# microsoft/DirectXTex

Hardware: AMD Instinct MI355X
Metric: Mtexels/s BC7 encode (4096^2 RGBA8, TEX_COMPRESS_DEFAULT) (higher is better)
Workload: dtype fp32 seed fit + i32 exact error sums (u8 texels in, 128-bit blocks out); 1 GPU; cfg2: 4096x4096 RGBA8 -> BC7_UNORM, TEX_COMPRESS_DEFAULT, one image per GPU, source and payload resident in HBM (dxtex_compress_device)

## Files before the change

directxtex_amd/csrc/bc6h_encode.hip:

```cpp
#include "dxtex_kernels.h"
#include "bc67_tables.h"
#include "bc7_core.h"
#include "bc6h_core.h"
#include "search_common.h"
#include <algorithm>
#include <cstdlib>
#include <cstdio>
#include <vector>

namespace dxtex
{
namespace
{
using namespace bc6h;

struct Ep16 { uint32_t a01, a2b0, b12; };
__device__ __forceinline__ Ep16 pack_ep16(const int (&A)[3], const int (&B)[3])
{
    Ep16 e;
    e.a01 = (uint32_t(A[0]) & 0xFFFFu) | (uint32_t(A[1]) << 16);
    e.a2b0 = (uint32_t(A[2]) & 0xFFFFu) | (uint32_t(B[0]) << 16);
    e.b12 = (uint32_t(B[1]) & 0xFFFFu) | (uint32_t(B[2]) << 16);
    return e;
}
// ... 24 lines not shown
    return s;
}
struct Rec6 { Ep16 ep; float err; };
struct Best6 { float err; uint32_t mode; uint64_t lo, hi; };
struct OrgSave { Ep16 ep; float err; uint64_t idx; };
struct OptSave { uint64_t idx; float err; uint32_t swapped; };

enum : int { SEED_INTS = 17 * 6 + 2 };

struct Bc6hArgs
{
    SegTable seg;
    uint32_t nblocks;
    int isSigned;
    int prune;
    uint32_t taskBase;
    int prec1[4];
    float* fpix;
    uint8_t* lists;
    int* seeds;
    Rec6* recs;
    OrgSave* orgs;
    uint2* order; uint32_t* tinfo; uint32_t* counters;
    Best6* best;
    float* bounds;
    int boundsReady;
    int filterStats;
    int samePrec;
    struct OptSave* opts;
    int saveOpt;
    ModeRt mode;
};

constexpr uint32_t kDoneBit6 = 1u << 23;

#if !defined(DXTEX_BC6H_DEFAULT_ORDER)
#define DXTEX_BC6H_DEFAULT_ORDER "5,6,7,8,0,2,3,4,1,9"
#endif

__device__ __forceinline__ Texels slot_texels(float* slot , int np)
{
    Texels t; t.r = slot; t.g = slot + 16 * 64; t.b = slot + 32 * 64; t.stride = 64; t.np = np;
    return t;
}

__device__ __forceinline__ int gather_texels(const float* planes, uint32_t mask, float* slot, uint64_t& pos)
// ... 921 lines not shown
        if (lane == 0)
        {
            a.recs[myTask].ep = pack_ep16(st.ep.A, st.ep.B);
            { const float mk = ep16_mark(sg, st.ep.A, st.ep.B); if (mk < 0.0f) a.recs[myTask].err = mk; }
        }
    }
}

__global__ void __launch_bounds__(256) bc6h_store_kernel(Bc6hArgs a)
{
    const uint32_t nb = blockIdx.x * 256u + threadIdx.x;
    if (nb >= a.nblocks) return;
    const Best6 b = a.best[nb];
    const BcSeg& im = seg_of(a.seg, nb);
    const uint32_t gb = im.nb0 + (nb - im.l0);
    const uint32_t by = gb / im.nbw, bx = gb - by * im.nbw;
    uint64_t* out = reinterpret_cast<uint64_t*>(im.dst + uint64_t(by) * im.dstRowPitch) + 2 * uint64_t(bx);
    out[0] = b.lo; out[1] = b.hi;
}

const uint64_t kMaxBlocksPerPass6 = dev_env("DXTEX_MAX_BLOCKS_PER_PASS") ? std::max<uint64_t>(1, strtoull(dev_env("DXTEX_MAX_BLOCKS_PER_PASS"), nullptr, 10)) : (1u << 22);
struct Scratch6
{
    size_t fpix, lists, seeds, recs, orgs, order, tinfo, counters, best, bounds, recs1, orgs1, order1, tinfo1, counters1, opts, total;
    explicit Scratch6(uint64_t nb)
    {
        auto up = [](size_t v) { return (v + 255) & ~size_t(255); };
        size_t o = 0;
        fpix = o; o = up(o + nb * 48 * sizeof(float));
        lists = o; o = up(o + nb * 8);
        seeds = o; o = up(o + nb * SEED_INTS * sizeof(int));
        recs = o; o = up(o + nb * 16 * sizeof(Rec6));
        orgs = o; o = up(o + nb * 16 * sizeof(OrgSave));
        order = o; o = up(o + nb * 16 * sizeof(uint2));
        tinfo = o; o = up(o + nb * 16 * sizeof(uint32_t));
        counters = o; o = up(o + 128 * sizeof(uint32_t));
        best = o; o = up(o + nb * sizeof(Best6));
        bounds = o; o = up(o + nb * 17 * sizeof(float));
        recs1 = o; o = up(o + nb * 4 * sizeof(Rec6));
        orgs1 = o; o = up(o + nb * 4 * sizeof(OrgSave));
        order1 = o; o = up(o + nb * 4 * sizeof(uint2));
        tinfo1 = o; o = up(o + nb * 4 * sizeof(uint32_t));
        counters1 = o; o = up(o + 128 * sizeof(uint32_t));
        opts = o; o = up(o + nb * 16 * sizeof(OptSave));
        total = o;
    }
};
}

size_t bc6h_scratch_bytes(uint64_t nblocks, size_t nimages)
{
    return Scratch6(nblocks < kMaxBlocksPerPass6 ? nblocks : kMaxBlocksPerPass6).total + seg_table_bytes(nblocks, kMaxBlocksPerPass6, nimages);
}

hipError_t launch_bc6h_encode(const SrcView& src, uint8_t* dst, uint64_t dstRowPitch, bool isSigned, void* scratch,
                              hipStream_t stream, KernelMarks* marks, const SideStreams* side)
{
    BcImage one; one.src = src; one.dst = dst; one.dstRowPitch = dstRowPitch;
    return launch_bc6h_encode_many(&one, 1, isSigned, scratch, stream, marks, side);
}

hipError_t launch_bc6h_encode_many(const BcImage* images, size_t count, bool isSigned, void* scratch, hipStream_t stream, KernelMarks* marks,
                                   const SideStreams* side)
{
#define DXTEX_MARK(NAME) do { if (marks) marks->mark(NAME); } while (0)
    std::vector<BcSeg> segs;
// ... 1 lines not shown
    uint64_t perPass = 0;
    if (!build_passes(images, count, kMaxBlocksPerPass6, segs, passes, &perPass)) return hipSuccess;
    const Scratch6 L(perPass);
    uint8_t* base = static_cast<uint8_t*>(scratch);
    BcSeg* dSegs = reinterpret_cast<BcSeg*>(base + L.total);
    const hipError_t ce = upload_segments(dSegs, segs, passes, stream);
    if (ce != hipSuccess) return ce;
    for (const BcPass& pass : passes)
    {
        Bc6hArgs a;
        set_pass(a.seg, dSegs, segs, pass);
        a.nblocks = pass.nblocks;
        a.isSigned = isSigned ? 1 : 0;
        static const bool noPrune = dev_env("DXTEX_BC6H_NO_PRUNE") != nullptr;
        a.prune = noPrune ? 0 : 1;
        a.fpix = reinterpret_cast<float*>(base + L.fpix);
        a.lists = base + L.lists;
        a.seeds = reinterpret_cast<int*>(base + L.seeds);
        a.recs = reinterpret_cast<Rec6*>(base + L.recs);
        a.orgs = reinterpret_cast<OrgSave*>(base + L.orgs);
        a.order = reinterpret_cast<uint2*>(base + L.order);
        a.tinfo = reinterpret_cast<uint32_t*>(base + L.tinfo);
        a.counters = reinterpret_cast<uint32_t*>(base + L.counters);
        a.best = reinterpret_cast<Best6*>(base + L.best);
        a.bounds = reinterpret_cast<float*>(base + L.bounds);
        a.opts = reinterpret_cast<OptSave*>(base + L.opts);
        a.saveOpt = 0;
        a.boundsReady = 0;
        a.filterStats = 0;
        a.mode = ModeRt();

        DXTEX_MARK("bc6h_rough");
        hipLaunchKernelGGL(bc6h_rough_kernel, dim3((a.nblocks + 3) / 4), dim3(256), 0, stream, a);
        DXTEX_MARK("bc6h_block_seed");
        hipLaunchKernelGGL(bc6h_block_seed_kernel, dim3((a.nblocks + 255) / 256), dim3(256), 0, stream, a);
        if (dev_env("DXTEX_BC6H_DUMP"))
        {
            (void)hipStreamSynchronize(stream);
            const uint32_t n = std::min<uint32_t>(a.nblocks, 4);
            std::vector<uint8_t> l(n * 8); std::vector<int> sd(n * SEED_INTS);
            (void)hipMemcpy(l.data(), a.lists, l.size(), hipMemcpyDeviceToHost);
            (void)hipMemcpy(sd.data(), a.seeds, sd.size() * 4, hipMemcpyDeviceToHost);
            for (uint32_t b = 0; b < n; ++b)
            {
                fprintf(stderr, "block %u shapes:", b);
                for (int i = 0; i < 8; ++i) fprintf(stderr, " %d", l[b * 8 + i]);
                fprintf(stderr, "\n  seeds rank0:");
                for (int i = 0; i < 12; ++i) fprintf(stderr, " %d", sd[b * SEED_INTS + i]);
                fprintf(stderr, "\n");
            }
        }
        static const int onlyMode = dev_env("DXTEX_BC6H_ONLY_MODE") ? atoi(dev_env("DXTEX_BC6H_ONLY_MODE")) : -1;
        static const bool noSearch = dev_env("DXTEX_BC6H_NO_SEARCH") != nullptr;
        static const Bc6hMode kModes[14] = {
            { 0x00, 1, 1, 3, { 10, 10, 10 }, { 5, 5, 5 } }, { 0x01, 1, 1, 3, { 7, 7, 7 }, { 6, 6, 6 } }, { 0x02, 1, 1, 3, { 11, 11, 11 }, { 5, 4, 4 } },
            { 0x06, 1, 1, 3, { 11, 11, 11 }, { 4, 5, 4 } }, { 0x0a, 1, 1, 3, { 11, 11, 11 }, { 4, 4, 5 } }, { 0x0e, 1, 1, 3, { 9, 9, 9 }, { 5, 5, 5 } },
            { 0x12, 1, 1, 3, { 8, 8, 8 }, { 6, 5, 5 } }, { 0x16, 1, 1, 3, { 8, 8, 8 }, { 5, 6, 5 } }, { 0x1a, 1, 1, 3, { 8, 8, 8 }, { 5, 5, 6 } },
            { 0x1e, 1, 0, 3, { 6, 6, 6 }, { 6, 6, 6 } }, { 0x03, 0, 0, 4, { 10, 10, 10 }, { 10, 10, 10 } }, { 0x07, 0, 1, 4, { 11, 11, 11 }, { 9, 9, 9 } },
            { 0x0b, 0, 1, 4, { 12, 12, 12 }, { 8, 8, 8 } }, { 0x0f, 0, 1, 4, { 16, 16, 16 }, { 4, 4, 4 } } };
        auto set_mode_on = [&](Bc6hArgs& a, int mi)
        {
            const Bc6hMode& k = kModes[mi];
            a.mode.index = mi; a.mode.code = k.code; a.mode.regions2 = k.regions2; a.mode.transformed = k.transformed; a.mode.prec = k.prec[0];
            for (int c = 0; c < 3; ++c) a.mode.delta[c] = k.delta[c];
        };
        auto set_mode = [&](int mi) { set_mode_on(a, mi); };
        auto sort_tasks = [&](const Bc6hArgs& a, uint32_t ntasks, hipStream_t stream)
        {
            const uint32_t binGroups = std::min<uint32_t>(kBinGroups, (ntasks + 255) / 256);
            (void)hipMemsetAsync(a.counters, 0, 128 * sizeof(uint32_t), stream);
            hipLaunchKernelGGL(bc7_bin_count_kernel, dim3(binGroups), dim3(256), 0, stream, a.tinfo, ntasks, a.counters);
            hipLaunchKernelGGL(bc7_bin_scan_kernel, dim3(1), dim3(1), 0, stream, a.counters);
            hipLaunchKernelGGL(bc7_bin_scatter_kernel, dim3(binGroups), dim3(256), 0, stream, a.tinfo, ntasks, a.counters, a.order);
        };
        a.taskBase = 0;
        for (int m = 0; m < 4; ++m) a.prec1[m] = kModes[10 + m].prec[0];
        static const std::vector<int> order6 = []
        {
            std::vector<int> o;
            const char* e = dev_env("DXTEX_BC6H_ORDER");
            const char* p = e ? e : DXTEX_BC6H_DEFAULT_ORDER;
            while (*p) { if (*p >= '0' && *p <= '9') o.push_back(int(strtol(p, const_cast<char**>(&p), 10))); else ++p; }
            return o;
        }();
        int prevPrec = -1;
        a.samePrec = 0;
        std::vector<int> run2;
        for (int mi : order6) if (mi >= 0 && mi <= 9 && (onlyMode < 0 || mi == onlyMode)) run2.push_back(mi);
        static const int forkBack = dev_env("DXTEX_BC6H_FORK_BACK") ? atoi(dev_env("DXTEX_BC6H_FORK_BACK")) : 2;
        const SideStreams* fork = (marks || forkBack <= 0 || run2.size() < size_t(forkBack) + 1 || onlyMode >= 0) ? nullptr : side;
        Bc6hArgs a1 = a;
        a1.recs = reinterpret_cast<Rec6*>(base + L.recs1);
        a1.orgs = reinterpret_cast<OrgSave*>(base + L.orgs1);
        a1.order = reinterpret_cast<uint2*>(base + L.order1);
        a1.tinfo = reinterpret_cast<uint32_t*>(base + L.tinfo1);
        a1.counters = reinterpret_cast<uint32_t*>(base + L.counters1);
        a1.samePrec = 0;
        auto one_region_search = [&](hipStream_t stream, KernelMarks* marks)
        {
            const uint32_t gridPP = (a1.nblocks + 255) / 256;
            DXTEX_MARK("bc6h_pre_1region");
            a1.boundsReady = 0;
            for (int m = 0; m < 4; ++m)
            {
                if (onlyMode >= 0 && 10 + m != onlyMode) continue;
                set_mode_on(a1, 10 + m); a1.taskBase = uint32_t(m) * a1.nblocks;
                hipLaunchKernelGGL(bc6h_pre_kernel<0>, dim3(gridPP), dim3(256), 0, stream, a1);
                a1.boundsReady = 1;
            }
            const uint32_t ntasks = a1.nblocks * 4u;
            if (onlyMode >= 0)
                for (int m = 0; m < 4; ++m) if (10 + m != onlyMode) (void)hipMemsetAsync(a1.tinfo + uint64_t(m) * a1.nblocks, 0, uint64_t(a1.nblocks) * 4, stream);
            DXTEX_MARK("bc6h_bin_1region");
            sort_tasks(a1, ntasks, stream);
            DXTEX_MARK("bc6h_perturb_1region");
            static const uint32_t waveMax = dev_env("DXTEX_BC6H_WAVE_MAX") ? uint32_t(strtoul(dev_env("DXTEX_BC6H_WAVE_MAX"), nullptr, 0)) : kWaveTaskMax6;
            if (!noSearch)
            {
                hipLaunchKernelGGL(bc6h_perturb_kernel<16>, dim3(std::min<uint32_t>(kSearchWaves, (ntasks + 63) / 64)), dim3(64), 0, stream, a1, waveMax);
                hipLaunchKernelGGL(bc6h_perturb_wave_kernel, dim3(std::min<uint32_t>(kSearchWaves, ntasks)), dim3(64), 0, stream, a1, waveMax);
            }
        };
        bool forked = false;
        for (size_t at = 0; at < run2.size(); ++at)
        {
            const int mi = run2[at];
            if (fork && at + size_t(forkBack) == run2.size())
            {
                (void)hipEventRecord(fork->forked, stream);
                (void)hipStreamWaitEvent(fork->side[0], fork->forked, 0);
                one_region_search(fork->side[0], nullptr);
                (void)hipEventRecord(fork->joined[0], fork->side[0]);
                forked = true;
            }
            set_mode(mi);
            static const bool noReuse = dev_env("DXTEX_BC6H_NO_REUSE") != nullptr;
            a.samePrec = (!noReuse && prevPrec == kModes[mi].prec[0]) ? 1 : 0;
            prevPrec = kModes[mi].prec[0];
            a.saveOpt = (!noReuse && at + 1 < run2.size() && kModes[run2[at + 1]].prec[0] == kModes[mi].prec[0]) ? 1 : 0;
            const uint32_t ntasks = a.nblocks * 16u;
            const uint32_t gridPP = (a.nblocks + 15) / 16;
            static const char* const kPre[10] = { "bc6h_pre_m0", "bc6h_pre_m1", "bc6h_pre_m2", "bc6h_pre_m3", "bc6h_pre_m4", "bc6h_pre_m5", "bc6h_pre_m6", "bc6h_pre_m7", "bc6h_pre_m8", "bc6h_pre_m9" };
            static const char* const kPerturb[10] = { "bc6h_perturb_m0", "bc6h_perturb_m1", "bc6h_perturb_m2", "bc6h_perturb_m3", "bc6h_perturb_m4", "bc6h_perturb_m5", "bc6h_perturb_m6", "bc6h_perturb_m7", "bc6h_perturb_m8", "bc6h_perturb_m9" };
            static const char* const kPost[10] = { "bc6h_post_m0", "bc6h_post_m1", "bc6h_post_m2", "bc6h_post_m3", "bc6h_post_m4", "bc6h_post_m5", "bc6h_post_m6", "bc6h_post_m7", "bc6h_post_m8", "bc6h_post_m9" };
            DXTEX_MARK(kPre[mi]);
            hipLaunchKernelGGL(bc6h_pre_kernel<1>, dim3(gridPP), dim3(256), 0, stream, a);
            a.boundsReady = 1;
            DXTEX_MARK("bc6h_bin_2region");
            sort_tasks(a, ntasks, stream);
#if defined(DXTEX_DEV)
            static const bool stats6 = dev_env("DXTEX_BC6H_STATS") != nullptr;
            a.filterStats = stats6 ? 1 : 0;
            if (stats6)
            {
                uint32_t c[40] = {};
                (void)hipStreamSynchronize(stream);
                (void)hipMemcpy(c, a.counters, sizeof(c), hipMemcpyDeviceToHost);
                std::fprintf(stderr, "bc6h stats mode %d (prec %d): %u task slots, %u live (16-texel: %u)\n", mi, a.mode.prec, ntasks, c[34], c[16]);
            }
#endif
            DXTEX_MARK(kPerturb[mi]);
            static const bool plainPerturb = dev_env("DXTEX_BC6H_PERTURB_PLAIN") != nullptr;
            if (!noSearch)
            {
                const dim3 grid(std::min<uint32_t>(kSearchWaves, (ntasks + 63) / 64));
                if (plainPerturb) hipLaunchKernelGGL(bc6h_perturb_kernel<8>, grid, dim3(64), 0, stream, a, 0u);
                else if (isSigned) hipLaunchKernelGGL(bc6h_perturb_filter_kernel<true>, grid, dim3(64), 0, stream, a);
                else hipLaunchKernelGGL(bc6h_perturb_filter_kernel<false>, grid, dim3(64), 0, stream, a);
            }
#if defined(DXTEX_DEV)
            if (stats6 && !plainPerturb)
            {
// ... 41 lines not shown
```

directxtex_amd/csrc/bc7_encode.hip:

```cpp
#include "dxtex_kernels.h"
#include "bc67_tables.h"
#include "bc7_core.h"
#include "search_common.h"
#include <algorithm>
#include <cstdio>
#include <cstdlib>
#include <vector>

namespace dxtex
{
namespace
{
using namespace bc7;

struct Cand { uint32_t err; uint32_t ord; uint64_t lo, hi; };

enum : int { SLOT_M0 = 0, SLOT_M1, SLOT_M2, SLOT_M3, SLOT_M4A, SLOT_M4B, SLOT_M5, SLOT_M6, SLOT_M7, NUM_SLOTS };
enum : int { LIST_BYTES = 64 };

enum : int { PHASE_ALL = 0, PHASE_EARLY = 1, PHASE_LATE = 2 };

struct Bc7Args
{
    SegTable seg;
    uint32_t nblocks;
    uint32_t flags;
    uint8_t* lists;
    Cand* cands;
    uint32_t* px;
    struct TaskRec* recs;
    uint2* order;
    uint32_t* tinfo;
    uint32_t* counters;
    uint32_t* zeroOrd;
    uint2* seeds1;
    uint2* seeds3;
    uint2* seeds;
    int* bestErr;
    int prune;
    const uint32_t* flagged;
    uint32_t early6Min;
    uint32_t earlyAlphaMin;
    int early6Pct;
    int phase;
    const uint32_t* gate;
    uint32_t gateMin;
    uint32_t perturbWaveMax;
    uint32_t exhWaveMax;
};

constexpr uint32_t kWaveTaskMax = 262144;
constexpr uint32_t kWaveTaskMax45 = 24576;
constexpr uint32_t kPerturbWaveMax = 32768;

__device__ __forceinline__ void load_block_texel(const SrcView& src, uint32_t nbw, uint32_t nb, uint32_t t, float* f4, uint32_t& ldr)
{
// ... 336 lines not shown
template<int MODE, int IM>
__device__ __forceinline__ void search_pickup(const Bc7Args& a, uint2 task, uint32_t* slotCol, SlotRegion& rg)
{
    typedef TaskMap<MODE, IM> TM;
    const uint32_t nb = task.x / TM::TPB;
    const uint32_t mask = task.y & 0xFFFFu, rot = (task.y >> 16) & 3u;
    const uint4* px4 = reinterpret_cast<const uint4*>(a.px + uint64_t(nb) * 16);
    const uint4 q0 = px4[0], q1 = px4[1], q2 = px4[2], q3 = px4[3];
    const uint32_t px[16] = { q0.x, q0.y, q0.z, q0.w, q1.x, q1.y, q1.z, q1.w, q2.x, q2.y, q2.z, q2.w, q3.x, q3.y, q3.z, q3.w };
    int np = 0;
    if (TM::NS == 1)
    {
#pragma unroll
        for (int i = 0; i < 16; ++i) slotCol[i * kSlotStride] = rotate_pixel(px[i], rot);
        np = 16;
    }
    else
    {
#pragma unroll
        for (int i = 0; i < 16; ++i)
            if ((mask >> i) & 1u) { slotCol[np * kSlotStride] = px[i]; ++np; }
    }
    rg.base = slotCol; rg.np = np; rg.p2sum = 0;
}

__device__ __forceinline__ int lanes_below(unsigned long long mask)
{
    return int(__builtin_amdgcn_mbcnt_hi(uint32_t(mask >> 32), __builtin_amdgcn_mbcnt_lo(uint32_t(mask), 0u)));
}

#if defined(DXTEX_BC7_WAVETIMES)
enum : int { WT_KINDS = 3, WT_KEYS = WT_KINDS * 8 * 2 * 3, WT_FIELDS = 6 };
__device__ unsigned long long g_wt[WT_KEYS][8192][WT_FIELDS];
__device__ unsigned int g_wtHist[WT_KEYS][256];
#define WT_BEGIN(KIND) const int wtKey = (((KIND) * 8 + MODE) * 2 + IM) * 3 + CHSET; const bool wtOn = a.phase != PHASE_EARLY; \
    const unsigned long long wt0 = wall_clock64(); unsigned long long wtDr = 0, wtRounds = 0, wtLanes = 0, wtTasks = 0; int wtMine = 0
#define WT_TAKE(IDX) do { wtTasks += (unsigned long long)__popcll(__ballot((IDX) != 0xFFFFFFFFu)); if (!wtDr && q.drained) wtDr = wall_clock64(); } while (0)
#define WT_ROUND(BUSYL) do { ++wtRounds; wtLanes += (unsigned long long)__popcll(__ballot(BUSYL)); if (BUSYL) ++wtMine; } while (0)
#define WT_DONE() do { wtMine = 0; } while (0)
#define WT_END() do { if (wtOn && lane == 0 && wtRounds) { unsigned long long* w_ = g_wt[wtKey][blockIdx.x & 8191]; w_[0] = wt0; w_[1] = wtDr ? wtDr : wall_clock64(); \
    w_[2] = wall_clock64(); w_[3] = wtRounds; w_[4] = wtLanes; w_[5] = wtTasks; } } while (0)
#else
#define WT_BEGIN(KIND) do { } while (0)
#define WT_TAKE(IDX) do { } while (0)
#define WT_ROUND(BUSYL) do { } while (0)
#define WT_DONE() do { } while (0)
#define WT_END() do { } while (0)
#endif
#if !defined(DXTEX_FLAT_SKIP)
#define DXTEX_FLAT_SKIP 1
#endif
// ... 840 lines not shown
    {
        if (!((slotMask >> s) & 1u)) continue;
        if (s == SLOT_M7 && a.flagged[1] == 0) continue;
        const Cand v = c[s];
        if (v.err == 0xFFFFFFFFu) continue;
        const uint64_t key = (uint64_t(v.err) << 32) | v.ord;
        if (key < bestKey) { bestKey = key; lo = v.lo; hi = v.hi; }
    }
    const BcSeg& sg = seg_of(a.seg, nb);
    const uint32_t gb = sg.nb0 + (nb - sg.l0);
    const uint32_t by = gb / sg.nbw, bx = gb - by * sg.nbw;
    uint64_t* out = reinterpret_cast<uint64_t*>(sg.dst + uint64_t(by) * sg.dstRowPitch) + 2 * uint64_t(bx);
    out[0] = lo; out[1] = hi;
}
}

namespace
{
const uint64_t kMaxBlocksPerPass = dev_env("DXTEX_MAX_BLOCKS_PER_PASS") ? std::max<uint64_t>(1, strtoull(dev_env("DXTEX_MAX_BLOCKS_PER_PASS"), nullptr, 10)) : (1u << 22);
constexpr int kMaxTasksPerBlock = 64;
const uint64_t kSmallPassBlocks = dev_env("DXTEX_BC7_SMALL_BLOCKS") ? strtoull(dev_env("DXTEX_BC7_SMALL_BLOCKS"), nullptr, 10) : 262144;
struct ScratchLayout
{
    size_t lists, cands, px, recs, order, tinfo, counters, zeroOrd, bestErr, seeds, seeds1, seeds3, flagcnt, auxRecs, auxOrder, auxTinfo, auxCounters, total;
    size_t auxTpb, auxSlices;
    explicit ScratchLayout(uint64_t nb, bool threeSubsets)
    {
        auto up = [](size_t v) { return (v + 255) & ~size_t(255); };
        const size_t tpb = threeSubsets ? kMaxTasksPerBlock : 32;
        const bool small = nb <= kSmallPassBlocks;
        auxTpb = small ? tpb : 4; auxSlices = small ? size_t(kSideStreams) : 2;
        size_t o = 0;
        lists = o; o = up(o + nb * LIST_BYTES);
        cands = o; o = up(o + nb * NUM_SLOTS * sizeof(Cand));
        px = o; o = up(o + nb * 64);
        recs = o; o = up(o + nb * tpb * sizeof(TaskRec));
        order = o; o = up(o + nb * tpb * sizeof(uint2));
        tinfo = o; o = up(o + nb * tpb * sizeof(uint32_t));
        counters = o; o = up(o + 64 * sizeof(uint32_t));
        zeroOrd = o; o = up(o + nb * sizeof(uint32_t));
        bestErr = o; o = up(o + nb * sizeof(int));
        seeds = o; o = up(o + nb * 64 * sizeof(uint2));
        seeds1 = o; o = up(o + nb * 2 * sizeof(uint2));
        seeds3 = o; o = up(o + (threeSubsets ? nb * 192 * sizeof(uint2) : 0));
        flagcnt = o; o = up(o + 256);
        auxRecs = o; o = up(o + auxSlices * nb * auxTpb * sizeof(TaskRec));
        auxOrder = o; o = up(o + auxSlices * nb * auxTpb * sizeof(uint2));
        auxTinfo = o; o = up(o + auxSlices * nb * auxTpb * sizeof(uint32_t));
        auxCounters = o; o = up(o + size_t(kSideStreams) * 64 * sizeof(uint32_t));
        total = o;
    }
};

template<int MODE, int IM>
void launch_mode(const Bc7Args& a0, hipStream_t stream, KernelMarks* marks, const char* const (&names)[7])
{
    typedef TaskMap<MODE, IM> TM;
    constexpr int BPW = (TM::TPB >= 64) ? 1 : 64 / TM::TPB;
    const uint32_t nb = a0.nblocks;
    const uint32_t ntasks = nb * uint32_t(TM::TPB);
    const uint32_t gridPP = (nb + 4 * BPW - 1) / (4 * BPW);
    constexpr bool kWhole = TM::NS == 1;
    constexpr uint32_t kExhMax = (MODE == 6) ? kWaveTaskMax : kWaveTaskMax45;
    static const bool noGroup = dev_env("DXTEX_BC7_NO_GROUP") != nullptr;
    const bool maybeShortP = kWhole && !noGroup && (MODE == 6 || ntasks <= 4u * kPerturbWaveMax);
    const bool maybeShortE = kWhole && !noGroup && (MODE == 6 || ntasks <= 4u * kExhMax);
    const uint32_t wavesP = std::min<uint32_t>(kSearchWaves, (ntasks + 1) / 2), wavesE = std::min<uint32_t>(kSearchWaves, ntasks);
    Bc7Args a = a0;
    a.gate = nullptr; a.gateMin = 0;
    if (a0.flagged && !(a0.flags & BCF_BC7_QUICK))
    {
        if (MODE == 7) { a.gate = a0.flagged + 1; a.gateMin = 1; }
        else if (a0.phase == PHASE_EARLY && (MODE == 4 || MODE == 5)) { a.gate = a0.flagged + 1; a.gateMin = std::max<uint32_t>(1u, a0.earlyAlphaMin); }
        else if (a0.phase == PHASE_EARLY && MODE == 6) { a.gate = a0.flagged; a.gateMin = std::max<uint32_t>(1u, a0.early6Min); }
    }
    a.perturbWaveMax = maybeShortP ? kPerturbWaveMax : 0u;
    a.exhWaveMax = maybeShortE ? kExhMax : 0u;
    if (marks) marks->mark(names[0]);
    hipLaunchKernelGGL((bc7_pre_kernel<MODE, IM>), dim3(gridPP), dim3(256), 0, stream, a);
    if (marks) marks->mark(names[1]);
    (void)hipMemsetAsync(a.counters, 0, 64 * sizeof(uint32_t), stream);
    const uint32_t binGroups = std::min<uint32_t>(kBinGroups, (ntasks + 255) / 256);
    hipLaunchKernelGGL(bc7_bin_count_kernel, dim3(binGroups), dim3(256), 0, stream, a.tinfo, ntasks, a.counters, a.gate, a.gateMin);
    hipLaunchKernelGGL(bc7_bin_scan_kernel, dim3(1), dim3(1), 0, stream, a.counters);
    hipLaunchKernelGGL(bc7_bin_scatter_kernel, dim3(binGroups), dim3(256), 0, stream, a.tinfo, ntasks, a.counters, a.order, a.gate, a.gateMin);
    if (marks) marks->mark(names[2]);
    const uint32_t waves = std::min<uint32_t>(kSearchWaves, (ntasks + 63) / 64);
    static const int tailBelow = dev_env("DXTEX_BC7_TAIL_BELOW") ? atoi(dev_env("DXTEX_BC7_TAIL_BELOW")) : 48;
    static const bool perturbPlain = dev_env("DXTEX_BC7_PERTURB_PLAIN") != nullptr;
    static const int rangeTests = dev_env("DXTEX_BC7_NO_PEEL") ? 3 : ((dev_env("DXTEX_BC7_RANGE_TESTS") ? atoi(dev_env("DXTEX_BC7_RANGE_TESTS")) & 0xFF : DXTEX_RANGE_TESTS) |
                                                                       ((dev_env("DXTEX_BC7_PEEL_LAYERS") ? atoi(dev_env("DXTEX_BC7_PEEL_LAYERS")) : 1) << 8));
    if constexpr (PaletteBits<MODE, IM>::AB == 0)
    {
        if constexpr (MODE == 1 || MODE == 6)
        {
            if (perturbPlain) hipLaunchKernelGGL((bc7_perturb_kernel<MODE, IM, CH_ALL>), dim3(waves), dim3(64), 0, stream, a, 0);
            else hipLaunchKernelGGL((bc7_perturb_filter_kernel<MODE, IM, CH_ALL>), dim3(waves), dim3(64), 0, stream, a, 0);
        }
        else
            hipLaunchKernelGGL((bc7_perturb_kernel<MODE, IM, CH_ALL>), dim3(waves), dim3(64), 0, stream, a, 0);
        if constexpr (kWhole) { if (maybeShortP) hipLaunchKernelGGL((bc7_perturb_wave_kernel<MODE, IM, CH_ALL>), dim3(wavesP), dim3(64), 0, stream, a); }
        if (marks) marks->mark(names[4]);
        if constexpr (kWhole) { if (maybeShortE) hipLaunchKernelGGL((bc7_exhaustive_wave_kernel<MODE, IM, CH_ALL>), dim3(wavesE), dim3(64), 0, stream, a); }
        hipLaunchKernelGGL((bc7_exhaustive_kernel<MODE, IM, CH_ALL>), dim3(waves), dim3(64), 0, stream, a, 1, tailBelow, rangeTests);
    }
    else
    {
        if constexpr (MODE == 4 && IM == 1 && DXTEX_PF_M4 != 0)
// ... 124 lines not shown
    const bool three = (flags & BCF_USE_3SUBSETS) != 0;
    const ScratchLayout L(perPass, three);
    uint8_t* base = static_cast<uint8_t*>(scratch);
    BcSeg* dSegs = reinterpret_cast<BcSeg*>(base + L.total);
    const hipError_t ce = upload_segments(dSegs, segs, passes, stream);
    if (ce != hipSuccess) return ce;
    const bool quick = (flags & BCF_BC7_QUICK) != 0;

    for (const BcPass& pass : passes)
    {
        Bc7Args a;
        set_pass(a.seg, dSegs, segs, pass);
        a.nblocks = pass.nblocks;
        a.flags = flags;
        a.perturbWaveMax = 0; a.exhWaveMax = 0;
        a.gate = nullptr; a.gateMin = 0;
        a.lists = base + L.lists;
        a.cands = reinterpret_cast<Cand*>(base + L.cands);
        a.px = reinterpret_cast<uint32_t*>(base + L.px);
        a.recs = reinterpret_cast<TaskRec*>(base + L.recs);
        a.order = reinterpret_cast<uint2*>(base + L.order);
        a.tinfo = reinterpret_cast<uint32_t*>(base + L.tinfo);
        a.counters = reinterpret_cast<uint32_t*>(base + L.counters);
        a.zeroOrd = reinterpret_cast<uint32_t*>(base + L.zeroOrd);
        a.bestErr = reinterpret_cast<int*>(base + L.bestErr);
        a.seeds = reinterpret_cast<uint2*>(base + L.seeds);
        a.seeds1 = reinterpret_cast<uint2*>(base + L.seeds1);
        a.seeds3 = reinterpret_cast<uint2*>(base + L.seeds3);
        static const bool noPrune = dev_env("DXTEX_BC7_NO_PRUNE") != nullptr;
        a.prune = noPrune ? 0 : 1;
        static const int early6 = dev_env("DXTEX_BC7_EARLY6_PCT") ? atoi(dev_env("DXTEX_BC7_EARLY6_PCT")) : 100;
        a.early6Pct = early6;
        uint32_t slotMask = 0;

        uint32_t* flagCount = reinterpret_cast<uint32_t*>(base + L.flagcnt);
        a.flagged = flagCount;
        static const int early6MinPct = dev_env("DXTEX_BC7_EARLY6_MIN_PCT") ? atoi(dev_env("DXTEX_BC7_EARLY6_MIN_PCT")) : -1;
        static const int earlyAlphaMinPct = dev_env("DXTEX_BC7_EARLYA_MIN_PCT") ? atoi(dev_env("DXTEX_BC7_EARLYA_MIN_PCT")) : 25;
        const bool smallPlanRuns = side && !marks && !quick && dev_env("DXTEX_BC7_SERIAL") == nullptr && dev_env("DXTEX_BC7_NO_SMALL_PLAN") == nullptr &&
                                   L.auxTpb >= 32 && perPass <= kSmallPassBlocks && dev_env("DXTEX_BC7_ORDER") == nullptr;
        a.early6Min = uint32_t(uint64_t(a.nblocks) * uint32_t(early6MinPct >= 0 ? early6MinPct : (smallPlanRuns ? 25 : 50)) / 100u);
        a.earlyAlphaMin = uint32_t(uint64_t(a.nblocks) * uint32_t(earlyAlphaMinPct) / 100u);
        if (!quick)
        {
            DXTEX_MARK("bc7_rough");
            hipLaunchKernelGGL(bc7_rough_kernel, dim3((a.nblocks + 3) / 4), dim3(256), 0, stream, a);
// ... 37 lines not shown
            case 8: DXTEX_MODE(4, 1, "mode4_im1"); slotMask |= 1u << SLOT_M4B; break;
            case 18: DXTEX_MODE(4, 1, "mode4_im1_early"); slotMask |= 1u << SLOT_M4B; break;
            case 28: DXTEX_MODE(4, 1, "mode4_im1_late"); slotMask |= 1u << SLOT_M4B; break;
            case 5: DXTEX_MODE(5, 0, "mode5"); slotMask |= 1u << SLOT_M5; break;
            case 15: DXTEX_MODE(5, 0, "mode5_early"); slotMask |= 1u << SLOT_M5; break;
            case 25: DXTEX_MODE(5, 0, "mode5_late"); slotMask |= 1u << SLOT_M5; break;
            case 6: DXTEX_MODE(6, 0, "mode6"); slotMask |= 1u << SLOT_M6; break;
            case 16: DXTEX_MODE(6, 0, "mode6_early"); slotMask |= 1u << SLOT_M6; break;
            case 26: DXTEX_MODE(6, 0, "mode6_late"); slotMask |= 1u << SLOT_M6; break;
            case 7: DXTEX_MODE(7, 0, "mode7"); slotMask |= 1u << SLOT_M7; break;
            default: break;
            }
        };
        auto family45 = [](int step) { const int m = step % 10; return m == 4 || m == 8 || m == 5; };
        static const bool serial45 = dev_env("DXTEX_BC7_SERIAL") != nullptr;
        const SideStreams* fork = (marks || serial45 || quick) ? nullptr : side;
        auto side_args = [&](const Bc7Args& a0, size_t k)
        {
            Bc7Args b = a0;
            b.recs = reinterpret_cast<TaskRec*>(base + L.auxRecs) + k * size_t(a0.nblocks) * L.auxTpb;
            b.order = reinterpret_cast<uint2*>(base + L.auxOrder) + k * size_t(a0.nblocks) * L.auxTpb;
            b.tinfo = reinterpret_cast<uint32_t*>(base + L.auxTinfo) + k * size_t(a0.nblocks) * L.auxTpb;
            b.counters = reinterpret_cast<uint32_t*>(base + L.auxCounters) + k * 64;
            return b;
        };
        static const std::vector<std::vector<std::vector<int>>> smallPlan = []
        {
            const char* e = dev_env("DXTEX_BC7_SMALL_PLAN");
            const char* p = e ? e : "1,26/3,2/16,14,15,18,7,0|24/28/25";
            std::vector<std::vector<std::vector<int>>> stages(1, std::vector<std::vector<int>>(1));
            while (*p)
            {
                if (*p >= '0' && *p <= '9') stages.back().back().push_back(int(strtol(p, const_cast<char**>(&p), 10)));
                else
                {
                    if (*p == '|') stages.emplace_back(1);
                    else if (*p == '/' && stages.back().size() < size_t(kSideStreams) + 1) stages.back().emplace_back();
                    ++p;
                }
            }
            return stages;
        }();
        static const bool noSmall = dev_env("DXTEX_BC7_NO_SMALL_PLAN") != nullptr;
        if (fork && !noSmall && smallPlanRuns)
        {
            for (const std::vector<std::vector<int>>& stage : smallPlan)
// ... 53 lines not shown
```

directxtex_amd/csrc/search_common.h:

```cpp
#pragma once
#include <hip/hip_runtime.h>
#include <stdint.h>
#include <algorithm>
#include <cstring>
#include <vector>
#include "dxtex_kernels.h"

namespace dxtex
{
namespace
{
struct BcSeg
{
    SrcView src;
    uint8_t* dst;
    uint64_t dstRowPitch;
    uint32_t nbw;
    uint32_t nb0;
    uint32_t l0;
    uint32_t pad;
};

struct SegTable
{
// ... 100 lines not shown
    return v;
}

__device__ __forceinline__ void selection_pass(int& e, uint32_t& s, int lane, int i)
{
    const int v = (lane >= i) ? e : 0x7FFFFFFF;
    const int incl = wave_prefix_min(v);
    int excl = __builtin_amdgcn_update_dpp(0x7FFFFFFF, incl, 0x138, 0xF, 0xF, false);
    if (lane <= i) excl = 0x7FFFFFFF;
    const bool isrec = (lane > i) && (e < excl);
    const unsigned long long mask = __ballot(isrec);
    int srcLane = lane;
    if (isrec)
    {
        const unsigned long long below = mask & ((1ull << lane) - 1ull);
        srcLane = below ? (63 - __clzll(below)) : i;
    }
    else if (lane == i && mask)
        srcLane = 63 - __clzll(mask);
    e = __shfl(e, srcLane);
    s = uint32_t(__shfl(int(s), srcLane));
}

constexpr int kBinGroups = 2048;

__global__ void __launch_bounds__(256) bc7_bin_count_kernel(const uint32_t* tinfo, uint32_t ntasks, uint32_t* counters, const uint32_t* gate = nullptr, uint32_t gateMin = 0)
{
    if (gate && *gate < gateMin) return;
    __shared__ uint32_t hist[17];
    if (threadIdx.x < 17) hist[threadIdx.x] = 0;
    __syncthreads();
    const uint32_t per = (ntasks + gridDim.x - 1) / gridDim.x;
    const uint32_t t0 = blockIdx.x * per, t1 = min(ntasks, t0 + per);
    for (uint32_t t = t0 + threadIdx.x; t < t1; t += 256)
    {
        const uint32_t np = tinfo[t] >> 24;
        if (np) atomicAdd(&hist[np], 1u);
    }
    __syncthreads();
    if (threadIdx.x >= 1 && threadIdx.x <= 16 && hist[threadIdx.x]) atomicAdd(&counters[threadIdx.x], hist[threadIdx.x]);
}

__global__ void bc7_bin_scan_kernel(uint32_t* counters)
{
    if (threadIdx.x != 0 || blockIdx.x != 0) return;
    uint32_t run = 0;
    for (int b = 16; b >= 1; --b) { counters[17 + b] = run; run += counters[b]; }
    counters[34] = run;
}

__global__ void __launch_bounds__(256) bc7_bin_scatter_kernel(const uint32_t* tinfo, uint32_t ntasks, uint32_t* counters, uint2* order, const uint32_t* gate = nullptr, uint32_t gateMin = 0)
{
    if (gate && *gate < gateMin) return;
    __shared__ uint32_t hist[17], cursor[17];
    if (threadIdx.x < 17) hist[threadIdx.x] = 0;
    __syncthreads();
    const uint32_t per = (ntasks + gridDim.x - 1) / gridDim.x;
    const uint32_t t0 = blockIdx.x * per, t1 = min(ntasks, t0 + per);
    for (uint32_t t = t0 + threadIdx.x; t < t1; t += 256)
    {
        const uint32_t np = tinfo[t] >> 24;
        if (np) atomicAdd(&hist[np], 1u);
    }
    __syncthreads();
    if (threadIdx.x >= 1 && threadIdx.x <= 16)
        cursor[threadIdx.x] = hist[threadIdx.x] ? atomicAdd(&counters[17 + threadIdx.x], hist[threadIdx.x]) : 0u;
    __syncthreads();
    for (uint32_t t = t0 + threadIdx.x; t < t1; t += 256)
    {
        const uint32_t ti = tinfo[t], np = ti >> 24;
        if (np) order[atomicAdd(&cursor[np], 1u)] = make_uint2(t, ti);
    }
}

constexpr int kQueueBase = 36;
constexpr int kSearchWaves = 8192;

constexpr uint32_t kQueueBatch = 128;

struct WaveQueue
{
    uint32_t lo, hi;
    bool drained;
};

__device__ __forceinline__ uint32_t queue_take(WaveQueue& q, uint32_t* head, uint32_t live, unsigned long long idle, int lane)
{
    if (q.lo >= q.hi && !q.drained)
    {
        const uint32_t batch = (live > uint32_t(kSearchWaves) * 64u) ? kQueueBatch : 64u;
        uint32_t base = 0;
        if (lane == 0) base = atomicAdd(head, batch);
        base = uint32_t(__builtin_amdgcn_readfirstlane(int(base)));
        q.lo = base;
        q.hi = min(base + batch, live);
// ... 12 lines not shown
```

Measured before the change: 136.4 Mtexels/s.

## Replace atomic task binning with deterministic wave-ballot count/scatter sort

```diff
diff --git a/directxtex_amd/csrc/bc6h_encode.hip b/directxtex_amd/csrc/bc6h_encode.hip
--- a/directxtex_amd/csrc/bc6h_encode.hip
+++ b/directxtex_amd/csrc/bc6h_encode.hip
@@ -70,6 +70,7 @@
     Rec6* recs;
     OrgSave* orgs;
     uint2* order; uint32_t* tinfo; uint32_t* counters;
+    uint32_t* bins;
     Best6* best;
     float* bounds;
     int boundsReady;
@@ -1037,7 +1038,7 @@
 const uint64_t kMaxBlocksPerPass6 = dev_env("DXTEX_MAX_BLOCKS_PER_PASS") ? std::max<uint64_t>(1, strtoull(dev_env("DXTEX_MAX_BLOCKS_PER_PASS"), nullptr, 10)) : (1u << 22);
 struct Scratch6
 {
-    size_t fpix, lists, seeds, recs, orgs, order, tinfo, counters, best, bounds, recs1, orgs1, order1, tinfo1, counters1, opts, total;
+    size_t fpix, lists, seeds, recs, orgs, order, tinfo, counters, bins, best, bounds, recs1, orgs1, order1, tinfo1, counters1, bins1, opts, total;
     explicit Scratch6(uint64_t nb)
     {
         auto up = [](size_t v) { return (v + 255) & ~size_t(255); };
@@ -1050,6 +1051,7 @@
         order = o; o = up(o + nb * 16 * sizeof(uint2));
         tinfo = o; o = up(o + nb * 16 * sizeof(uint32_t));
         counters = o; o = up(o + 128 * sizeof(uint32_t));
+        bins = o; o = up(o + kBinScratchWords * sizeof(uint32_t));
         best = o; o = up(o + nb * sizeof(Best6));
         bounds = o; o = up(o + nb * 17 * sizeof(float));
         recs1 = o; o = up(o + nb * 4 * sizeof(Rec6));
@@ -1057,6 +1059,7 @@
         order1 = o; o = up(o + nb * 4 * sizeof(uint2));
         tinfo1 = o; o = up(o + nb * 4 * sizeof(uint32_t));
         counters1 = o; o = up(o + 128 * sizeof(uint32_t));
+        bins1 = o; o = up(o + kBinScratchWords * sizeof(uint32_t));
         opts = o; o = up(o + nb * 16 * sizeof(OptSave));
         total = o;
     }
@@ -1104,6 +1107,7 @@
         a.order = reinterpret_cast<uint2*>(base + L.order);
         a.tinfo = reinterpret_cast<uint32_t*>(base + L.tinfo);
         a.counters = reinterpret_cast<uint32_t*>(base + L.counters);
+        a.bins = reinterpret_cast<uint32_t*>(base + L.bins);
         a.best = reinterpret_cast<Best6*>(base + L.best);
         a.bounds = reinterpret_cast<float*>(base + L.bounds);
         a.opts = reinterpret_cast<OptSave*>(base + L.opts);
@@ -1147,13 +1151,9 @@
             for (int c = 0; c < 3; ++c) a.mode.delta[c] = k.delta[c];
         };
         auto set_mode = [&](int mi) { set_mode_on(a, mi); };
-        auto sort_tasks = [&](const Bc6hArgs& a, uint32_t ntasks, hipStream_t stream)
-        {
-            const uint32_t binGroups = std::min<uint32_t>(kBinGroups, (ntasks + 255) / 256);
-            (void)hipMemsetAsync(a.counters, 0, 128 * sizeof(uint32_t), stream);
-            hipLaunchKernelGGL(bc7_bin_count_kernel, dim3(binGroups), dim3(256), 0, stream, a.tinfo, ntasks, a.counters);
-            hipLaunchKernelGGL(bc7_bin_scan_kernel, dim3(1), dim3(1), 0, stream, a.counters);
-            hipLaunchKernelGGL(bc7_bin_scatter_kernel, dim3(binGroups), dim3(256), 0, stream, a.tinfo, ntasks, a.counters, a.order);
+        auto sort_mode = [&](const Bc6hArgs& a, uint32_t ntasks, hipStream_t stream)
+        {
+            sort_tasks(a.tinfo, ntasks, a.counters, 128, a.bins, a.order, stream);
         };
         a.taskBase = 0;
         for (int m = 0; m < 4; ++m) a.prec1[m] = kModes[10 + m].prec[0];
@@ -1177,6 +1177,7 @@
         a1.order = reinterpret_cast<uint2*>(base + L.order1);
         a1.tinfo = reinterpret_cast<uint32_t*>(base + L.tinfo1);
         a1.counters = reinterpret_cast<uint32_t*>(base + L.counters1);
+        a1.bins = reinterpret_cast<uint32_t*>(base + L.bins1);
         a1.samePrec = 0;
         auto one_region_search = [&](hipStream_t stream, KernelMarks* marks)
         {
@@ -1194,7 +1195,7 @@
             if (onlyMode >= 0)
                 for (int m = 0; m < 4; ++m) if (10 + m != onlyMode) (void)hipMemsetAsync(a1.tinfo + uint64_t(m) * a1.nblocks, 0, uint64_t(a1.nblocks) * 4, stream);
             DXTEX_MARK("bc6h_bin_1region");
-            sort_tasks(a1, ntasks, stream);
+            sort_mode(a1, ntasks, stream);
             DXTEX_MARK("bc6h_perturb_1region");
             static const uint32_t waveMax = dev_env("DXTEX_BC6H_WAVE_MAX") ? uint32_t(strtoul(dev_env("DXTEX_BC6H_WAVE_MAX"), nullptr, 0)) : kWaveTaskMax6;
             if (!noSearch)
@@ -1229,7 +1230,7 @@
             hipLaunchKernelGGL(bc6h_pre_kernel<1>, dim3(gridPP), dim3(256), 0, stream, a);
             a.boundsReady = 1;
             DXTEX_MARK("bc6h_bin_2region");
-            sort_tasks(a, ntasks, stream);
+            sort_mode(a, ntasks, stream);
 #if defined(DXTEX_DEV)
             static const bool stats6 = dev_env("DXTEX_BC6H_STATS") != nullptr;
             a.filterStats = stats6 ? 1 : 0;
diff --git a/directxtex_amd/csrc/bc7_encode.hip b/directxtex_amd/csrc/bc7_encode.hip
--- a/directxtex_amd/csrc/bc7_encode.hip
+++ b/directxtex_amd/csrc/bc7_encode.hip
@@ -32,6 +32,7 @@
     uint2* order;
     uint32_t* tinfo;
     uint32_t* counters;
+    uint32_t* bins;
     uint32_t* zeroOrd;
     uint2* seeds1;
     uint2* seeds3;
@@ -414,11 +415,6 @@
             if ((mask >> i) & 1u) { slotCol[np * kSlotStride] = px[i]; ++np; }
     }
     rg.base = slotCol; rg.np = np; rg.p2sum = 0;
-}
-
-__device__ __forceinline__ int lanes_below(unsigned long long mask)
-{
-    return int(__builtin_amdgcn_mbcnt_hi(uint32_t(mask >> 32), __builtin_amdgcn_mbcnt_lo(uint32_t(mask), 0u)));
 }
 
 #if defined(DXTEX_BC7_WAVETIMES)
@@ -1305,7 +1301,7 @@
 const uint64_t kSmallPassBlocks = dev_env("DXTEX_BC7_SMALL_BLOCKS") ? strtoull(dev_env("DXTEX_BC7_SMALL_BLOCKS"), nullptr, 10) : 262144;
 struct ScratchLayout
 {
-    size_t lists, cands, px, recs, order, tinfo, counters, zeroOrd, bestErr, seeds, seeds1, seeds3, flagcnt, auxRecs, auxOrder, auxTinfo, auxCounters, total;
+    size_t lists, cands, px, recs, order, tinfo, counters, bins, zeroOrd, bestErr, seeds, seeds1, seeds3, flagcnt, auxRecs, auxOrder, auxTinfo, auxCounters, auxBins, total;
     size_t auxTpb, auxSlices;
     explicit ScratchLayout(uint64_t nb, bool threeSubsets)
     {
@@ -1321,6 +1317,7 @@
         order = o; o = up(o + nb * tpb * sizeof(uint2));
         tinfo = o; o = up(o + nb * tpb * sizeof(uint32_t));
         counters = o; o = up(o + 64 * sizeof(uint32_t));
+        bins = o; o = up(o + kBinScratchWords * sizeof(uint32_t));
         zeroOrd = o; o = up(o + nb * sizeof(uint32_t));
         bestErr = o; o = up(o + nb * sizeof(int));
         seeds = o; o = up(o + nb * 64 * sizeof(uint2));
@@ -1331,6 +1328,7 @@
         auxOrder = o; o = up(o + auxSlices * nb * auxTpb * sizeof(uint2));
         auxTinfo = o; o = up(o + auxSlices * nb * auxTpb * sizeof(uint32_t));
         auxCounters = o; o = up(o + size_t(kSideStreams) * 64 * sizeof(uint32_t));
+        auxBins = o; o = up(o + size_t(kSideStreams) * kBinScratchWords * sizeof(uint32_t));
         total = o;
     }
 };
@@ -1362,11 +1360,7 @@
     if (marks) marks->mark(names[0]);
     hipLaunchKernelGGL((bc7_pre_kernel<MODE, IM>), dim3(gridPP), dim3(256), 0, stream, a);
     if (marks) marks->mark(names[1]);
-    (void)hipMemsetAsync(a.counters, 0, 64 * sizeof(uint32_t), stream);
-    const uint32_t binGroups = std::min<uint32_t>(kBinGroups, (ntasks + 255) / 256);
-    hipLaunchKernelGGL(bc7_bin_count_kernel, dim3(binGroups), dim3(256), 0, stream, a.tinfo, ntasks, a.counters, a.gate, a.gateMin);
-    hipLaunchKernelGGL(bc7_bin_scan_kernel, dim3(1), dim3(1), 0, stream, a.counters);
-    hipLaunchKernelGGL(bc7_bin_scatter_kernel, dim3(binGroups), dim3(256), 0, stream, a.tinfo, ntasks, a.counters, a.order, a.gate, a.gateMin);
+    sort_tasks(a.tinfo, ntasks, a.counters, 64, a.bins, a.order, stream, a.gate, a.gateMin);
     if (marks) marks->mark(names[2]);
     const uint32_t waves = std::min<uint32_t>(kSearchWaves, (ntasks + 63) / 64);
     static const int tailBelow = dev_env("DXTEX_BC7_TAIL_BELOW") ? atoi(dev_env("DXTEX_BC7_TAIL_BELOW")) : 48;
@@ -1537,6 +1531,7 @@
         a.order = reinterpret_cast<uint2*>(base + L.order);
         a.tinfo = reinterpret_cast<uint32_t*>(base + L.tinfo);
         a.counters = reinterpret_cast<uint32_t*>(base + L.counters);
+        a.bins = reinterpret_cast<uint32_t*>(base + L.bins);
         a.zeroOrd = reinterpret_cast<uint32_t*>(base + L.zeroOrd);
         a.bestErr = reinterpret_cast<int*>(base + L.bestErr);
         a.seeds = reinterpret_cast<uint2*>(base + L.seeds);
@@ -1620,6 +1615,7 @@
             b.order = reinterpret_cast<uint2*>(base + L.auxOrder) + k * size_t(a0.nblocks) * L.auxTpb;
             b.tinfo = reinterpret_cast<uint32_t*>(base + L.auxTinfo) + k * size_t(a0.nblocks) * L.auxTpb;
             b.counters = reinterpret_cast<uint32_t*>(base + L.auxCounters) + k * 64;
+            b.bins = reinterpret_cast<uint32_t*>(base + L.auxBins) + k * kBinScratchWords;
             return b;
         };
         static const std::vector<std::vector<std::vector<int>>> smallPlan = []
diff --git a/directxtex_amd/csrc/search_common.h b/directxtex_amd/csrc/search_common.h
--- a/directxtex_amd/csrc/search_common.h
+++ b/directxtex_amd/csrc/search_common.h
@@ -146,55 +146,127 @@
     s = uint32_t(__shfl(int(s), srcLane));
 }
 
-constexpr int kBinGroups = 2048;
-
-__global__ void __launch_bounds__(256) bc7_bin_count_kernel(const uint32_t* tinfo, uint32_t ntasks, uint32_t* counters, const uint32_t* gate = nullptr, uint32_t gateMin = 0)
+__device__ __forceinline__ int lanes_below(unsigned long long mask)
+{
+    return int(__builtin_amdgcn_mbcnt_hi(uint32_t(mask >> 32), __builtin_amdgcn_mbcnt_lo(uint32_t(mask), 0u)));
+}
+
+constexpr int kBinWaves = 16;
+constexpr int kBinUnroll = 8;
+constexpr uint32_t kBinGroups = 512;
+constexpr uint32_t kBinWaveOff = kBinGroups * 16;
+constexpr size_t kBinScratchWords = size_t(kBinGroups) * 16 * (1 + kBinWaves);
+
+inline uint32_t bin_groups(uint32_t ntasks)
+{
+    const uint32_t perGroup = uint32_t(kBinWaves * kBinUnroll * 64);
+    return std::max<uint32_t>(1u, std::min<uint32_t>(kBinGroups, (ntasks + perGroup - 1) / perGroup));
+}
+
+__device__ __forceinline__ void bin_slice(uint32_t ntasks, uint32_t w, uint32_t& t0, uint32_t& t1)
+{
+    const uint32_t nw = gridDim.x * kBinWaves;
+    const uint32_t per = (((ntasks + nw - 1) / nw) + 63u) & ~63u;
+    t0 = min(ntasks, w * per);
+    t1 = min(ntasks, t0 + per);
+}
+
+template<bool SCATTER>
+__device__ __forceinline__ void bin_wave(const uint32_t* tinfo, uint32_t t0, uint32_t t1, int lane, uint32_t& cur, uint2* order)
+{
+    for (uint32_t t = t0; t < t1; t += kBinUnroll * 64)
+    {
+        uint32_t ti[kBinUnroll];
+#pragma unroll
+        for (int k = 0; k < kBinUnroll; ++k) { const uint32_t i = t + uint32_t(k * 64 + lane); ti[k] = (i < t1) ? tinfo[i] : 0u; }
+#pragma unroll
+        for (int k = 0; k < kBinUnroll; ++k)
+        {
+            const uint32_t np = ti[k] >> 24;
+            unsigned long long pending = __ballot(np != 0);
+            while (pending)
+            {
+                const uint32_t s = uint32_t(__builtin_amdgcn_readlane(int(np), __ffsll((long long)pending) - 1));
+                const unsigned long long m = __ballot(np == s);
+                if (SCATTER && np == s)
+                    order[uint32_t(__builtin_amdgcn_readlane(int(cur), int(s))) + uint32_t(lanes_below(m))] = make_uint2(t + uint32_t(k * 64 + lane), ti[k]);
+                if (uint32_t(lane) == s) cur += uint32_t(__popcll(m));
+                pending &= ~m;
+            }
+        }
+    }
+}
+
+__global__ void __launch_bounds__(kBinWaves * 64) bin_count_kernel(const uint32_t* tinfo, uint32_t ntasks, uint32_t* bins, const uint32_t* gate = nullptr, uint32_t gateMin = 0)
 {
     if (gate && *gate < gateMin) return;
-    __shared__ uint32_t hist[17];
-    if (threadIdx.x < 17) hist[threadIdx.x] = 0;
+    __shared__ uint32_t sCnt[kBinWaves][16];
+    const int wave = int(threadIdx.x >> 6), lane = int(threadIdx.x & 63);
+    uint32_t t0, t1;
+    bin_slice(ntasks, blockIdx.x * kBinWaves + uint32_t(wave), t0, t1);
+    uint32_t cnt = 0;
+    bin_wave<false>(tinfo, t0, t1, lane, cnt, nullptr);
+    if (lane >= 1 && lane <= 16) sCnt[wave][lane - 1] = cnt;
     __syncthreads();
-    const uint32_t per = (ntasks + gridDim.x - 1) / gridDim.x;
-    const uint32_t t0 = blockIdx.x * per, t1 = min(ntasks, t0 + per);
-    for (uint32_t t = t0 + threadIdx.x; t < t1; t += 256)
-    {
-        const uint32_t np = tinfo[t] >> 24;
-        if (np) atomicAdd(&hist[np], 1u);
+    if (threadIdx.x < 16)
+    {
+        uint32_t run = 0;
+        for (int w = 0; w < kBinWaves; ++w)
+        {
+            bins[kBinWaveOff + (blockIdx.x * kBinWaves + uint32_t(w)) * 16 + threadIdx.x] = run;
+            run += sCnt[w][threadIdx.x];
+        }
+        bins[blockIdx.x * 16 + threadIdx.x] = run;
+    }
+}
+
+__global__ void __launch_bounds__(kBinWaves * 64) bin_scatter_kernel(const uint32_t* tinfo, uint32_t ntasks, const uint32_t* bins, uint32_t* counters, uint2* order,
+                                                                      const uint32_t* gate = nullptr, uint32_t gateMin = 0)
+{
+    if (gate && *gate < gateMin) return;
+    constexpr int kParts = kBinWaves * 4;
+    __shared__ uint32_t sTot[kParts][16], sPre[kParts][16], sBase[16];
+    const int wave = int(threadIdx.x >> 6), lane = int(threadIdx.x & 63);
+    {
+        const uint32_t b = threadIdx.x & 15u, p = threadIdx.x >> 4;
+        uint32_t tot = 0, pre = 0;
+        for (uint32_t h = p; h < gridDim.x; h += kParts) { const uint32_t v = bins[h * 16 + b]; tot += v; pre += (h < blockIdx.x) ? v : 0u; }
+        sTot[p][b] = tot; sPre[p][b] = pre;
     }
     __syncthreads();
-    if (threadIdx.x >= 1 && threadIdx.x <= 16 && hist[threadIdx.x]) atomicAdd(&counters[threadIdx.x], hist[threadIdx.x]);
-}
-
-__global__ void bc7_bin_scan_kernel(uint32_t* counters)
-{
-    if (threadIdx.x != 0 || blockIdx.x != 0) return;
-    uint32_t run = 0;
-    for (int b = 16; b >= 1; --b) { counters[17 + b] = run; run += counters[b]; }
-    counters[34] = run;
-}
-
-__global__ void __launch_bounds__(256) bc7_bin_scatter_kernel(const uint32_t* tinfo, uint32_t ntasks, uint32_t* counters, uint2* order, const uint32_t* gate = nullptr, uint32_t gateMin = 0)
-{
-    if (gate && *gate < gateMin) return;
-    __shared__ uint32_t hist[17], cursor[17];
-    if (threadIdx.x < 17) hist[threadIdx.x] = 0;
+    if (threadIdx.x < 16)
+    {
+        uint32_t tot = 0, pre = 0;
+        for (int p = 0; p < kParts; ++p) { tot += sTot[p][threadIdx.x]; pre += sPre[p][threadIdx.x]; }
+        sTot[0][threadIdx.x] = tot; sPre[0][threadIdx.x] = pre;
+    }
     __syncthreads();
-    const uint32_t per = (ntasks + gridDim.x - 1) / gridDim.x;
-    const uint32_t t0 = blockIdx.x * per, t1 = min(ntasks, t0 + per);
-    for (uint32_t t = t0 + threadIdx.x; t < t1; t += 256)
-    {
-        const uint32_t np = tinfo[t] >> 24;
-        if (np) atomicAdd(&hist[np], 1u);
+    if (threadIdx.x < 16)
+    {
+        uint32_t start = 0, live = 0;
+        for (int b = 0; b < 16; ++b) { live += sTot[0][b]; start += (b > int(threadIdx.x)) ? sTot[0][b] : 0u; }
+        sBase[threadIdx.x] = start + sPre[0][threadIdx.x];
+        if (blockIdx.x == 0)
+        {
+            counters[1 + threadIdx.x] = sTot[0][threadIdx.x];
+            if (threadIdx.x == 0) counters[34] = live;
+        }
     }
     __syncthreads();
-    if (threadIdx.x >= 1 && threadIdx.x <= 16)
-        cursor[threadIdx.x] = hist[threadIdx.x] ? atomicAdd(&counters[17 + threadIdx.x], hist[threadIdx.x]) : 0u;
-    __syncthreads();
-    for (uint32_t t = t0 + threadIdx.x; t < t1; t += 256)
-    {
-        const uint32_t ti = tinfo[t], np = ti >> 24;
-        if (np) order[atomicAdd(&cursor[np], 1u)] = make_uint2(t, ti);
-    }
+    uint32_t t0, t1;
+    bin_slice(ntasks, blockIdx.x * kBinWaves + uint32_t(wave), t0, t1);
+    uint32_t cur = 0;
+    if (lane >= 1 && lane <= 16) cur = sBase[lane - 1] + bins[kBinWaveOff + (blockIdx.x * kBinWaves + uint32_t(wave)) * 16 + uint32_t(lane - 1)];
+    bin_wave<true>(tinfo, t0, t1, lane, cur, order);
+}
+
+inline void sort_tasks(const uint32_t* tinfo, uint32_t ntasks, uint32_t* counters, size_t counterWords, uint32_t* bins, uint2* order, hipStream_t stream,
+                       const uint32_t* gate = nullptr, uint32_t gateMin = 0)
+{
+    (void)hipMemsetAsync(counters, 0, counterWords * sizeof(uint32_t), stream);
+    const uint32_t groups = bin_groups(ntasks);
+    hipLaunchKernelGGL(bin_count_kernel, dim3(groups), dim3(kBinWaves * 64), 0, stream, tinfo, ntasks, bins, gate, gateMin);
+    hipLaunchKernelGGL(bin_scatter_kernel, dim3(groups), dim3(kBinWaves * 64), 0, stream, tinfo, ntasks, bins, counters, order, gate, gateMin);
 }
 
 constexpr int kQueueBase = 36;
```

After: 136.2 Mtexels/s (median of 3 runs). No clear change (-0.1%).
